# mikel-brostrom/boxmot

Hardware: NVIDIA H100
Metric: tracker.update() frames/sec at 256 dets/frame (higher is better)
Workload: dtype bf16x3

## Files before the change

boxmot_b200/csrc/reid_tc.cuh:

```cuda
#pragma once
#include "wgmma.cuh"

namespace bmb {
namespace tcx {

typedef __nv_bfloat16 bf16;

__device__ __forceinline__ int tc_chunk_count(const int* d_n, int off, int cap) {
    int n = *d_n - off;
    n = n < 0 ? 0 : n;
    return n > cap ? cap : n;
}
using um::mbar_arrive;

__global__ void k_maxpool_planes(const float* __restrict__ in, int H, int W, int C, const int* __restrict__ d_n, int off,
                                 int cap, bf16* __restrict__ out_hi, bf16* __restrict__ out_lo) {
    const int n_crops = tc_chunk_count(d_n, off, cap);
    const int OH = H / 2, OW = W / 2, C8 = C / 8;
    const size_t total = (size_t)n_crops * C8 * OH * OW;
    for (size_t e = (size_t)blockIdx.x * blockDim.x + threadIdx.x; e < total; e += (size_t)gridDim.x * blockDim.x) {
        const int ox = (int)(e % OW);
        size_t r = e / OW;
        const int oy = (int)(r % OH); r /= OH;
        const int c8 = (int)(r % C8);
// ... 448 lines not shown
};
inline GemmSmem gemm_smem_layout(int K8, int NP, int NP2, int n_stage, bool tail, bool pool, int slot_bytes, bool pool2 = false) {
    GemmSmem s{};
    size_t o = 0;
    s.b = o; o += (size_t)K8 * 2 * NP * 16;
    s.b2 = o; if (tail) o += (size_t)(NP / 8) * 2 * NP2 * 16;
    o = (o + 127) & ~(size_t)127;
    s.ring = o; o += (size_t)n_stage * slot_bytes;
    s.a2 = o;
    if (tail) {
        size_t a2 = (size_t)2 * (NP / 8) * 128 * 16;
        if (pool2) a2 = a2 > (size_t)128 * (NP2 + 4) * 4 ? a2 : (size_t)128 * (NP2 + 4) * 4;
        o += a2;
    }
    s.f = pool2 ? s.a2 : o;
    if (pool) o += (size_t)128 * (NP + 4) * 4;
    s.gate = o; o += 4 * 32 * 4 + 64;
    s.total = o + 128;
    return s;
}

enum GemmMode { GM_PLAIN, GM_POOL, GM_TAIL, GM_TAIL_POOL2, GM_HEAD };

template <int NP, int NP2, int MODE>
constexpr int gemm_min_ctas() {
    return NP == 128 || ((MODE == GM_TAIL || MODE == GM_TAIL_POOL2) && NP >= 96) ? 1 : 2;
}

template <int NP, int NP2, int MODE>
__global__ void __launch_bounds__(GEMM_THREADS, (gemm_min_ctas<NP, NP2, MODE>()))
    k_gemm_tc(const __grid_constant__ GemmTcArgs a, const int* __restrict__ d_n, int off, int cap, const GemmSmem L, const GemmHeadIO hio) {
    constexpr bool tail = MODE == GM_TAIL || MODE == GM_TAIL_POOL2, pool = MODE == GM_POOL, pool2 = MODE == GM_TAIL_POOL2;
    static_assert(NP % 16 == 0 && NP >= 16 && NP <= 128, "NP: 16 .. 128 output channels");
    static_assert(tail ? (NP2 % 16 == 0 && NP2 >= 16 && NP2 <= 128) : NP2 == 0, "NP2: the tail's output channels");
    constexpr int NACC = (NP2 > NP ? NP2 : NP) / 2;
    const int n = blockIdx.y;
    if (n >= tc_chunk_count(d_n, off, cap)) return;
    extern __shared__ __align__(128) unsigned char smem[];
    __shared__ __align__(8) uint64_t bar_full[4], bar_empty[4], bar_w;
    const int warp = threadIdx.x >> 5, lane = threadIdx.x & 31;
    const int tile0 = blockIdx.x * a.tiles_per_cta;
    const int tile1 = min(tile0 + a.tiles_per_cta, a.tiles_per_crop);
    unsigned char* sB = smem + L.b;
    unsigned char* sB2 = smem + L.b2;
    unsigned char* sRing = smem + L.ring;
    unsigned char* sA2 = smem + L.a2;
    float* sF = reinterpret_cast<float*>(smem + L.f);

    if (threadIdx.x == 0) {
        for (int i = 0; i < a.n_stage; ++i) { um::mbar_init(&bar_full[i], 1); um::mbar_init(&bar_empty[i], 2); }
        um::mbar_init(&bar_w, 1);
        um::fence_mbar_init();
    }
    __syncthreads();

    if (warp == 8) {
        if (lane == 0) {
            {
                const uint32_t first = (uint32_t)((a.bfold ? 4 * a.midp : 0) / 8) * 2u * NP * 16u, total = (uint32_t)a.K8 * 2u * NP * 16u;
                const uint32_t b2 = tail ? (uint32_t)(NP / 8) * 2u * NP2 * 16u : 0u;
                um::mbar_expect_tx(&bar_w, total + b2);
                if (first) um::bulk_g2s(sB, reinterpret_cast<const unsigned char*>(a.bfold) + (size_t)n * first, first, &bar_w);
                if (total > first) um::bulk_g2s(sB + first, reinterpret_cast<const unsigned char*>(a.b_packed) + first, total - first, &bar_w);
                if (b2) um::bulk_g2s(sB2, a.b2_packed, b2, &bar_w);
            }
            uint32_t it = 0;
            for (int tile = tile0; tile < tile1; ++tile) {
                for (int s = 0; s < a.n_src; ++s) {
                    const int kc = a.src_kc[s];
                    for (int p0 = 0; p0 < a.src_planes[s]; p0 += kc, ++it) {
                        const uint32_t slot = it % (uint32_t)a.n_stage, ph = (it / (uint32_t)a.n_stage) & 1u;
                        um::mbar_wait(&bar_empty[slot], ph ^ 1u);
                        unsigned char* dst = sRing + (size_t)slot * a.slot_bytes;
                        um::mbar_expect_tx(&bar_full[slot], (uint32_t)kc * 128u * 16u * 2u);
                        um::tma_load_4d(dst, &a.map_hi[s], 0, tile * 2, p0, n, &bar_full[slot]);
                        um::tma_load_4d(dst + a.slot_bytes / 2, &a.map_lo[s], 0, tile * 2, p0, n, &bar_full[slot]);
                    }
                }
            }
        }
        return;
    }

    const int et = threadIdx.x;
    const int wg = warp >> 2;
    const int row = wg * 64 + (warp & 3) * 16 + (lane >> 2);
    const int cq = 2 * (lane & 3);
    const uint32_t lbo_b = 2u * NP * 16u, lo_off = (uint32_t)NP * 16u;
    um::mbar_wait(&bar_w, 0);
    float acc[NACC];
    uint32_t it = 0;
    for (int tile = tile0; tile < tile1; ++tile) {
        uint32_t kplane = 0, first = 1;
        uint32_t held = 0;
        for (int s = 0; s < a.n_src; ++s) {
            const int kc = a.src_kc[s];
            for (int p0 = 0; p0 < a.src_planes[s]; p0 += kc, ++it) {
                const uint32_t slot = it % (uint32_t)a.n_stage, ph = (it / (uint32_t)a.n_stage) & 1u;
                um::mbar_wait(&bar_full[slot], ph);
                const uint32_t ah = um::smem_u32(sRing + (size_t)slot * a.slot_bytes) + (uint32_t)wg * 1024u, al = ah + a.slot_bytes / 2;
                for (int ks = 0; ks < kc / 2; ++ks) {
                    const uint32_t bb = um::smem_u32(sB) + (kplane + 2 * ks) * lbo_b;
                    const uint64_t xh = um::make_desc(ah + ks * 2 * 2048u, 2048u, 128), xl = um::make_desc(al + ks * 2 * 2048u, 2048u, 128);
                    um::wg_fence();
                    um::mma<NP, false>(acc, xh, bb, lbo_b, 128, first ? 0u : 1u);
                    um::mma<NP, false>(acc, xl, bb, lbo_b, 128, 1u);
                    um::mma<NP, false>(acc, xh, bb + lo_off, lbo_b, 128, 1u);
                    first = 0;
                    um::wg_commit();
                    um::wg_wait<1>();
                    if (ks == 0 && kplane > 0 && (et & 127) == 0) mbar_arrive(&bar_empty[held]);
                }
                held = slot;
                kplane += kc;
            }
        }
        um::wg_wait<0>();
        um::wg_fence_acc<NACC>(acc);
        if ((et & 127) == 0) mbar_arrive(&bar_empty[held]);
        if constexpr (MODE == GM_HEAD) {
            um::bar_sync(1, 256);
            float* part = reinterpret_cast<float*>(sRing);
            float* pooled = part + 8 * NP;
            float* red = pooled + NP;
            float* feat = red + 8;
#pragma unroll
            for (int i = 0; i < NP / 8; ++i) {
                const int c = 8 * i + cq;
                const float2 b = *reinterpret_cast<const float2*>(a.bias + c);
                float o0 = fmaxf(acc[4 * i] + b.x, 0.f) + fmaxf(acc[4 * i + 2] + b.x, 0.f);
                float o1 = fmaxf(acc[4 * i + 1] + b.y, 0.f) + fmaxf(acc[4 * i + 3] + b.y, 0.f);
#pragma unroll
                for (int sh = 4; sh < 32; sh <<= 1) {
                    o0 += __shfl_xor_sync(0xffffffffu, o0, sh);
                    o1 += __shfl_xor_sync(0xffffffffu, o1, sh);
                }
                if (lane < 4) *reinterpret_cast<float2*>(part + warp * NP + c) = make_float2(o0, o1);
            }
            um::bar_sync(1, 256);
            for (int c = et; c < NP; c += 256)
                pooled[c] = (((part[c] + part[NP + c]) + (part[2 * NP + c] + part[3 * NP + c])) +
                             ((part[4 * NP + c] + part[5 * NP + c]) + (part[6 * NP + c] + part[7 * NP + c]))) / 128.f;
            um::bar_sync(1, 256);
            const int FEAT = a.head_feat, C = a.N;
            float sq = 0.f;
            for (int f = et; f < FEAT; f += 256) {
                float t[8] = {0.f, 0.f, 0.f, 0.f, 0.f, 0.f, 0.f, 0.f};
                int c = 0;
                for (; c + 8 <= C; c += 8) {
#pragma unroll
                    for (int u = 0; u < 8; ++u) t[u] = fmaf(pooled[c + u], a.head_w[(size_t)(c + u) * FEAT + f], t[u]);
                }
                for (; c < C; ++c) t[0] = fmaf(pooled[c], a.head_w[(size_t)c * FEAT + f], t[0]);
                float sv = a.head_b[f] + (((t[0] + t[1]) + (t[2] + t[3])) + ((t[4] + t[5]) + (t[6] + t[7])));
                sv = fmaxf(sv, 0.f);
                feat[f] = sv;
                sq = fmaf(sv, sv, sq);
            }
#pragma unroll
            for (int sh = 16; sh > 0; sh >>= 1) sq += __shfl_xor_sync(0xffffffffu, sq, sh);
            if (lane == 0) red[warp] = sq;
            um::bar_sync(1, 256);
            float tot = 0.f;
            for (int w = 0; w < 8; ++w) tot += red[w];
            const float nrm = sqrtf(tot);
            float* dst = hio.out + (size_t)hio.crops[off + n].out_row * hio.out_ld;
            for (int f = et; f < FEAT; f += 256) dst[f] = feat[f] / nrm;
            um::bar_sync(1, 256);
        } else {
#pragma unroll
            for (int i = 0; i < NP / 8; ++i) {
                const int c = 8 * i + cq;
                const float2 b = *reinterpret_cast<const float2*>(a.bias + c);
#pragma unroll
                for (int h = 0; h < 2; ++h) {
                    const int m = row + 8 * h, px = tile * 128 + m;
                    float o0 = acc[4 * i + 2 * h] + b.x, o1 = acc[4 * i + 2 * h + 1] + b.y;
                    if (a.relu) { o0 = fmaxf(o0, 0.f); o1 = fmaxf(o1, 0.f); }
                    if (a.out_f32) {
                        float* dst = a.out_f32 + ((size_t)n * a.HW + px) * a.N + c;
                        if (c + 1 < a.N) *reinterpret_cast<float2*>(dst) = make_float2(o0, o1);
                        else if (c < a.N) dst[0] = o0;
                    }
                    if constexpr (pool) {
                        *reinterpret_cast<float2*>(sF + (size_t)m * (NP + 4) + c) = make_float2(o0, o1);
                    } else if (a.out_hi || tail) {
                        uint32_t hv, lv;
                        um::split2(o0, o1, hv, lv);
                        if (a.out_hi) {
                            const size_t e = (((size_t)n * (NP / 8) + i) * a.HW + px) * 4 + (lane & 3);
                            reinterpret_cast<uint32_t*>(a.out_hi)[e] = hv;
                            reinterpret_cast<uint32_t*>(a.out_lo)[e] = lv;
                        }
                        if constexpr (tail) {
                            *reinterpret_cast<uint32_t*>(sA2 + ((size_t)i * 128 + m) * 16 + (lane & 3) * 4) = hv;
                            *reinterpret_cast<uint32_t*>(sA2 + ((size_t)(NP / 8 + i) * 128 + m) * 16 + (lane & 3) * 4) = lv;
                        }
                    }
                }
            }
            auto pool_store = [&](const int NPx, bf16* o_hi, bf16* o_lo) {
                um::bar_sync(1, 256);
                const int Wt = a.W, OW = Wt / 2, OHt = a.rows_per_tile / 2;
                const int items = OHt * OW * (NPx / 8);
                const int OHW = a.HW / 4;
                for (int e = et; e < items; e += 256) {
                    const int pp = e % (OHt * OW), c8 = e / (OHt * OW);
                    const int oy = pp / OW, ox = pp - oy * OW;
                    const float* f0 = sF + (size_t)((2 * oy) * Wt + 2 * ox) * (NPx + 4) + c8 * 8;
                    const float* f1 = f0 + (NPx + 4);
                    const float* f2 = f0 + (size_t)Wt * (NPx + 4);
                    const float* f3 = f2 + (NPx + 4);
                    uint32_t h[4], l[4];
#pragma unroll
                    for (int j = 0; j < 4; ++j) {
                        const float x0 = (f0[2 * j] + f1[2 * j] + f2[2 * j] + f3[2 * j]) * 0.25f;
                        const float x1 = (f0[2 * j + 1] + f1[2 * j + 1] + f2[2 * j + 1] + f3[2 * j + 1]) * 0.25f;
                        um::split2(x0, x1, h[j], l[j]);
                    }
                    const int opx = (tile * OHt + oy) * OW + ox;
                    const size_t o = ((size_t)n * (NPx / 8) + c8) * OHW + opx;
                    reinterpret_cast<uint4*>(o_hi)[o] = make_uint4(h[0], h[1], h[2], h[3]);
                    reinterpret_cast<uint4*>(o_lo)[o] = make_uint4(l[0], l[1], l[2], l[3]);
                }
                um::bar_sync(1, 256);
            };
            if constexpr (pool) pool_store(NP, a.out_hi, a.out_lo);
            if constexpr (tail) {
                um::fence_async_smem();
                um::bar_sync(2 + wg, 128);
                const uint32_t lbo_b2 = 2u * NP2 * 16u, lo2 = (uint32_t)NP2 * 16u;
                const uint32_t ah = um::smem_u32(sA2) + (uint32_t)wg * 1024u, al = ah + (uint32_t)(NP / 8) * 2048u;
                um::wg_fence();
                for (int ks = 0; ks < NP / 16; ++ks) {
                    const uint32_t bb = um::smem_u32(sB2) + ks * 2 * lbo_b2;
                    const uint64_t xh = um::make_desc(ah + ks * 2 * 2048u, 2048u, 128), xl = um::make_desc(al + ks * 2 * 2048u, 2048u, 128);
                    um::mma<NP2, false>(acc, xh, bb, lbo_b2, 128, ks > 0);
                    um::mma<NP2, false>(acc, xl, bb, lbo_b2, 128, 1u);
                    um::mma<NP2, false>(acc, xh, bb + lo2, lbo_b2, 128, 1u);
                }
                um::wg_commit();
                um::wg_wait<0>();
                um::wg_fence_acc<NACC>(acc);
                if constexpr (pool2) um::bar_sync(1, 256);
#pragma unroll
                for (int i = 0; i < NP2 / 8; ++i) {
                    const int c = 8 * i + cq;
                    const float2 b = *reinterpret_cast<const float2*>(a.bias2 + c);
#pragma unroll
                    for (int h = 0; h < 2; ++h) {
                        const int m = row + 8 * h, px = tile * 128 + m;
                        const float o0 = fmaxf(acc[4 * i + 2 * h] + b.x, 0.f), o1 = fmaxf(acc[4 * i + 2 * h + 1] + b.y, 0.f);
                        if constexpr (pool2) {
                            *reinterpret_cast<float2*>(sF + (size_t)m * (NP2 + 4) + c) = make_float2(o0, o1);
                        } else {
                            uint32_t hv, lv;
                            um::split2(o0, o1, hv, lv);
                            const size_t e = (((size_t)n * (NP2 / 8) + i) * a.HW + px) * 4 + (lane & 3);
                            reinterpret_cast<uint32_t*>(a.out2_hi)[e] = hv;
                            reinterpret_cast<uint32_t*>(a.out2_lo)[e] = lv;
                        }
                    }
                }
                if constexpr (pool2) pool_store(NP2, a.out2_hi, a.out2_lo);
            }
        }
    }
}

typedef void (*GemmKernel)(GemmTcArgs, const int*, int, int, GemmSmem, GemmHeadIO);
struct GemmInstance { int NP, NP2, mode; GemmKernel fn; };
#define BMB_GEMM(np, np2, mode) {np, np2, mode, k_gemm_tc<np, np2, mode>}
static const GemmInstance kGemmInstances[] = {
    BMB_GEMM(16, 0, GM_PLAIN), BMB_GEMM(32, 0, GM_PLAIN),
    BMB_GEMM(64, 0, GM_PLAIN), BMB_GEMM(96, 0, GM_PLAIN),
    BMB_GEMM(128, 0, GM_PLAIN),
    BMB_GEMM(64, 0, GM_POOL), BMB_GEMM(96, 0, GM_POOL),
    BMB_GEMM(64, 16, GM_TAIL), BMB_GEMM(96, 32, GM_TAIL), BMB_GEMM(128, 32, GM_TAIL),
    BMB_GEMM(64, 64, GM_TAIL_POOL2), BMB_GEMM(96, 96, GM_TAIL_POOL2),
    BMB_GEMM(128, 0, GM_HEAD),
};
#undef BMB_GEMM
inline GemmKernel gemm_instance(int NP, int NP2, int mode) {
    for (const GemmInstance& g : kGemmInstances)
        if (g.NP == NP && g.NP2 == NP2 && g.mode == mode) return g.fn;
    return nullptr;
}


struct FrontTcArgs {
    const uint8_t* images;
    size_t image_stride;
    int rows, cols;
    const void* crops;
    const bf16* w;
    const float* bias_tab;
    bf16* p_hi;
    bf16* p_lo;
    float* dbg_crop;
    int pad_mode;
};
struct FrontCrop { float x1, y1, x2, y2; int image, out_row; };

constexpr int FR_COLS = 39, FR_ROWS = 264, FR_CS = FR_ROWS * 8 + 16;
constexpr int FR_A_BYTES = FR_COLS * FR_CS;
constexpr int FR_W_BYTES = 7 * 4 * 32 * 16;
constexpr int FR_H_BYTES = 4 * 128 * 16 * 4;
constexpr size_t FR_SMEM = FR_A_BYTES + FR_W_BYTES + FR_H_BYTES + 128;

__device__ __forceinline__ void fr_coeff(int d, int src_n, double scale, bool clamp, int& idx, int& a0, int& a1) {
    float f = (float)(((double)d + 0.5) * scale - 0.5);
    int s = (int)floorf(f);
    f = f - (float)s;
    if (clamp) {
        if (s < 0) { s = 0; f = 0.f; }
        if (s >= src_n - 1) { s = src_n - 1; f = 0.f; }
    }
    idx = s;
    a0 = (int)rintf((1.0f - f) * 2048.0f);
    a1 = (int)rintf(f * 2048.0f);
}

__global__ void __launch_bounds__(256, 1) k_front_tc(const FrontTcArgs a, const int* __restrict__ d_n, int off, int cap) {
    const int n = blockIdx.y;
    if (n >= tc_chunk_count(d_n, off, cap)) return;
    const int strip = blockIdx.x;
    extern __shared__ __align__(128) unsigned char smem[];
    __shared__ int xi[128], xa0[128], xa1[128], yi[256], ya0[256], ya1[256];
    __shared__ __align__(16) float sBias[4 * 4 * 16];
    unsigned char* sA = smem;
    unsigned char* sW = smem + FR_A_BYTES;
    float* sH = reinterpret_cast<float*>(smem + FR_A_BYTES + FR_W_BYTES);
    const int warp = threadIdx.x >> 5, lane = threadIdx.x & 31;
    const FrontCrop cd = reinterpret_cast<const FrontCrop*>(a.crops)[off + n];
#ifdef BMB_TC_CLOCKS
    long long fk[16];
    int nfk = 0;
#define FCK() do { if (threadIdx.x == 0 && nfk < 16) fk[nfk++] = clock64(); } while (0)
#else
#define FCK() do { } while (0)
#endif
    FCK();

    const int x1 = (int)rintf(cd.x1), y1 = (int)rintf(cd.y1), x2 = (int)rintf(cd.x2), y2 = (int)rintf(cd.y2);
    const int cx1 = max(0, x1), cy1 = max(0, y1), cx2 = min(a.cols, x2), cy2 = min(a.rows, y2);
    const bool valid = cx2 > cx1 && cy2 > cy1;
    const int sw = cx2 - cx1, sh = cy2 - cy1;
    int nw = 128, nh = 256, pl = 0, pt = 0;
    if (valid && a.pad_mode) {
        const double sc = fmin(128.0 / (double)sw, 256.0 / (double)sh);
        nw = max(1, (int)((double)sw * sc));
        nh = max(1, (int)((double)sh * sc));
        pl = (128 - nw) / 2;
        pt = (256 - nh) / 2;
    }
    if (valid) {
        const double sx = 1.0 / ((double)nw / (double)sw), sy = 1.0 / ((double)nh / (double)sh);
        for (int d = threadIdx.x; d < nw; d += 256) fr_coeff(d, sw, sx, true, xi[d], xa0[d], xa1[d]);
        for (int d = threadIdx.x; d < nh; d += 256) fr_coeff(d, sh, sy, false, yi[d], ya0[d], ya1[d]);
    }
    for (int e = threadIdx.x; e < FR_A_BYTES / 16; e += 256) reinterpret_cast<uint4*>(sA)[e] = make_uint4(0u, 0u, 0u, 0u);
    for (int e = threadIdx.x; e < FR_W_BYTES / 16; e += 256) reinterpret_cast<uint4*>(sW)[e] = reinterpret_cast<const uint4*>(a.w)[e];
    for (int e = threadIdx.x; e < 256; e += 256) sBias[e] = a.bias_tab[e];
    __syncthreads();
    FCK();
    const int xin0 = 32 * strip - 5;
    if (valid) {
        const uint8_t* img = a.images + (size_t)cd.image * a.image_stride;
        for (int base = threadIdx.x; base < 40 * 256; base += 4 * 256) {
            int h0[4][3], h1[4][3], bb0[4], bb1[4], so[4];
            bool ok[4], border[4];
#pragma unroll
            for (int u = 0; u < 4; ++u) {
                const int p = base + u * 256;
                const int dy = p / 40, lc = p - dy * 40;
                const int dx = xin0 + lc;
                ok[u] = p < 40 * 256 && lc < FR_COLS && dx >= 0 && dx < 128;
                const int ry = dy - pt, rx = dx - pl;
                border[u] = rx < 0 || rx >= nw || ry < 0 || ry >= nh;
                const int dxc = min(max(rx, 0), nw - 1), dyc = min(max(ry, 0), nh - 1);
                const int sx0 = xi[dxc], sx1 = min(sx0 + 1, sw - 1);
                const int r0 = min(max(yi[dyc], 0), sh - 1), r1 = min(max(yi[dyc] + 1, 0), sh - 1);
                const uint8_t* p0 = img + ((size_t)(cy1 + r0) * a.cols + cx1) * 3;
                const uint8_t* p1 = img + ((size_t)(cy1 + r1) * a.cols + cx1) * 3;
                const int a0 = xa0[dxc], a1 = xa1[dxc];
                bb0[u] = ya0[dyc]; bb1[u] = ya1[dyc];
                so[u] = lc * FR_CS + (min(dy, 255) + 3) * 8;
#pragma unroll
                for (int c = 0; c < 3; ++c) {
                    h0[u][c] = (int)__ldg(p0 + sx0 * 3 + c) * a0 + (int)__ldg(p0 + sx1 * 3 + c) * a1;
                    h1[u][c] = (int)__ldg(p1 + sx0 * 3 + c) * a0 + (int)__ldg(p1 + sx1 * 3 + c) * a1;
                }
            }
#pragma unroll
            for (int u = 0; u < 4; ++u) {
                if (!ok[u]) continue;
                int v[3];
#pragma unroll
                for (int c = 0; c < 3; ++c) {
                    const int r = (((bb0[u] * (h0[u][c] >> 4)) >> 16) + ((bb1[u] * (h1[u][c] >> 4)) >> 16) + 2) >> 2;
                    v[c] = min(max(r, 0), 255);
                }
                if (border[u]) { v[0] = 104; v[1] = 116; v[2] = 124; }
                const __nv_bfloat162 rg = __floats2bfloat162_rn((float)v[2], (float)v[1]);
                const __nv_bfloat162 b_ = __floats2bfloat162_rn((float)v[0], 0.f);
                *reinterpret_cast<uint2*>(sA + so[u]) = make_uint2(*reinterpret_cast<const uint32_t*>(&rg), *reinterpret_cast<const uint32_t*>(&b_));
                if (a.dbg_crop) {
                    const int p = base + u * 256;
                    const int dy = p / 40, dx = xin0 + (p - dy * 40);
                    float* o = a.dbg_crop + (((size_t)n * 256 + dy) * 128 + dx) * 3;
                    o[0] = (float)v[2]; o[1] = (float)v[1]; o[2] = (float)v[0];
                }
            }
        }
    } else if (a.dbg_crop) {
        for (int p = threadIdx.x; p < 40 * 256; p += 256) {
            const int dy = p / 40, lc = p - dy * 40;
            const int dx = xin0 + lc;
            if (lc < FR_COLS && dx >= 0 && dx < 128) {
                float* o = a.dbg_crop + (((size_t)n * 256 + dy) * 128 + dx) * 3;
                o[0] = 0.f; o[1] = 0.f; o[2] = 0.f;
            }
        }
    }
    um::fence_async_smem();
    __syncthreads();
    FCK();

    const int wg = warp >> 2;
    const int row = wg * 64 + (warp & 3) * 16 + (lane >> 2);
    const int cq = 2 * (lane & 3);
    int rcl[2];
#pragma unroll
    for (int h = 0; h < 2; ++h) {
        const int oy = row + 8 * h;
        rcl[h] = oy == 0 ? 0 : (oy == 1 ? 1 : (oy == 127 ? 3 : 2));
    }
    float prev1[2][4], prev2[2][4];
#pragma unroll
    for (int h = 0; h < 2; ++h)
#pragma unroll
        for (int c = 0; c < 4; ++c) { prev1[h][c] = 0.f; prev2[h][c] = 0.f; }
    const uint32_t sa = um::smem_u32(sA) + (uint32_t)wg * 1024u, sw_ = um::smem_u32(sW);
    for (int j0 = 0; j0 < 17; j0 += 8) {
        const int j1 = min(j0 + 8, 17);
        for (int j = j0; j < j1; ++j) {
            const int ox = 16 * strip - 1 + j;
            float v[2][4];
            if (ox >= 0) {
                float acc[16];
                um::wg_fence();
#pragma unroll
                for (int kx = 0; kx < 7; ++kx)
#pragma unroll
                    for (int ks = 0; ks < 2; ++ks)
                        um::mma<32, false>(acc, um::make_desc(sa + (uint32_t)(2 * j + kx) * FR_CS + ks * 32, 16, 128),
                                           sw_ + (uint32_t)(kx * 4 + 2 * ks) * 512u, 512u, 128, (kx | ks) != 0);
                um::wg_commit();
                um::wg_wait_all();
                um::wg_fence_acc<16>(acc);
                const int cc = ox == 0 ? 0 : (ox == 1 ? 1 : (ox == 63 ? 3 : 2));
#pragma unroll
                for (int h = 0; h < 2; ++h) {
                    const float* bb = sBias + (rcl[h] * 4 + cc) * 16;
#pragma unroll
                    for (int i = 0; i < 2; ++i)
#pragma unroll
                        for (int e = 0; e < 2; ++e)
                            v[h][2 * i + e] = fmaxf(acc[4 * i + 2 * h + e] + acc[4 * (i + 2) + 2 * h + e] + bb[8 * i + cq + e], 0.f);
                }
            } else {
#pragma unroll
                for (int h = 0; h < 2; ++h)
#pragma unroll
                    for (int c = 0; c < 4; ++c) v[h][c] = 0.f;
            }
            if ((j & 1) == 0 && j >= 2) {
                float* hs = sH + (size_t)(((j - j0) >> 1) & 3) * 128 * 16;
#pragma unroll
                for (int h = 0; h < 2; ++h)
#pragma unroll
                    for (int i = 0; i < 2; ++i)
                        *reinterpret_cast<float2*>(hs + (row + 8 * h) * 16 + 8 * i + cq) =
                            make_float2(fmaxf(fmaxf(prev2[h][2 * i], prev1[h][2 * i]), v[h][2 * i]),
                                        fmaxf(fmaxf(prev2[h][2 * i + 1], prev1[h][2 * i + 1]), v[h][2 * i + 1]));
            }
#pragma unroll
            for (int h = 0; h < 2; ++h)
#pragma unroll
                for (int c = 0; c < 4; ++c) { prev2[h][c] = prev1[h][c]; prev1[h][c] = v[h][c]; }
        }
        __syncthreads();
        const int s_first = j0 == 0 ? 1 : 0, s_last = j0 == 0 ? 3 : (j0 == 8 ? 3 : 0);
        const int items = (s_last - s_first + 1) * 64 * 2;
        for (int e = threadIdx.x; e < items; e += 256) {
            const int s = s_first + (e >> 7), py = (e >> 1) & 63, half = e & 1;
            const float* hs = sH + (size_t)s * 128 * 16 + half * 8;
            const int oy = 2 * py;
            float m[8];
#pragma unroll
            for (int c = 0; c < 8; ++c) {
                const float up = oy > 0 ? hs[(oy - 1) * 16 + c] : 0.f;
                m[c] = fmaxf(fmaxf(up, hs[oy * 16 + c]), hs[(oy + 1) * 16 + c]);
            }
            const int px = 8 * strip + (j0 + 2 * s) / 2 - 1;
            uint32_t h4[4], l4[4];
#pragma unroll
            for (int c = 0; c < 4; ++c) um::split2(m[2 * c], m[2 * c + 1], h4[c], l4[c]);
            const size_t o = (((size_t)n * 2 + half) * 64 + py) * 32 + px;
            reinterpret_cast<uint4*>(a.p_hi)[o] = make_uint4(h4[0], h4[1], h4[2], h4[3]);
            reinterpret_cast<uint4*>(a.p_lo)[o] = make_uint4(l4[0], l4[1], l4[2], l4[3]);
        }
        __syncthreads();
        FCK();
    }
#ifdef BMB_TC_CLOCKS
    if (threadIdx.x == 0 && n == 5) {
        printf("front strip %d: setup %lld resize %lld |", strip, fk[1] - fk[0], fk[2] - fk[1]);
        for (int i = 3; i < nfk; ++i) printf(" batch %lld |", fk[i] - fk[i - 1]);
        printf(" total %lld\n", fk[nfk - 1] - fk[0]);
    }
#endif
}

}
}
```

boxmot_b200/csrc/reid_tc_plan.cuh:

```cuda
#pragma once

namespace bmb {
namespace tcx {

struct ChainShape { int CP, CR, W, H, R, kind; };
static const ChainShape kChainShapes[3] = {{16, 16, 32, 64, chain_rows<BMB_CHAIN_S2>(), LK_CHAIN_S2}, {32, 24, 16, 32, chain_rows<BMB_CHAIN_S3>(), LK_CHAIN_S3},
                                           {32, 32, 8, 16, chain_rows<BMB_CHAIN_S4>(), LK_CHAIN_S4}};

inline bool plan_supported(const ReidModel* m) {
    return m->arch == 1 && m->c[0] == 16 && m->c[1] == 64 && m->c[2] == 96 && m->c[3] == 128;
}

Plan* plan_build(ReidModel* m, const float* hw) {
    Plan* P = new Plan();
    try {
        P->chunk = m->chunk;
        const size_t CH = (size_t)m->chunk;
        int dev = 0;
        RCUDA_OK(cudaGetDevice(&dev));
        RCUDA_OK(cudaDeviceGetAttribute(&P->smem_limit, cudaDevAttrMaxSharedMemoryPerBlockOptin, dev));
        P->smem_limit -= 1024;
        alloc_planes(P->P, CH * 2048 * 16);
        alloc_planes(P->X1, CH * 2048 * 16);
        alloc_planes(P->Y, CH * 2048 * 64);
        alloc_planes(P->XA, CH * 2048 * 64);
        alloc_planes(P->XB, CH * 2048 * 64);
        RCUDA_OK(cudaMalloc(&P->c5, sizeof(float) * CH * 128 * m->c[3]));
        for (int b = 0; b < 4; ++b) RCUDA_OK(cudaMalloc(&P->sums[b], sizeof(float) * CH * 8 * 32));
        RCUDA_OK(cudaMalloc(&P->gates, sizeof(float) * CH * 4 * 32));
        RCUDA_OK(cudaMalloc(&P->arrivals, sizeof(int) * CH));
        RCUDA_OK(cudaMemset(P->arrivals, 0, sizeof(int) * CH));
        RCUDA_OK(cudaMalloc(&P->bfold, (size_t)CH * 16 * 2 * 128 * 16));
        RCUDA_OK(cudaMalloc(&P->dbg, sizeof(float) * CH * 2048 * 64));

        std::vector<uint16_t> wb;
        std::vector<float> wf;
        struct BlkOff { size_t pw[10], dw[10], lb[10], c1, c1b, cx, cxb; } bo[6];
        for (int bi = 0; bi < 6; ++bi) {
            const BlockW& b = m->blocks[bi];
            const int midp = pad16(b.mid);
            for (int l = 0; l < 10; ++l) {
                bo[bi].pw[l] = pack_b(wb, hw + b.light[l].pw, b.mid, b.mid, b.mid, midp / 8, midp);
                size_t at = (wf.size() + 3) / 4 * 4;
                wf.resize(at + 9 * midp, 0.f);
                for (int t = 0; t < 9; ++t)
                    for (int c = 0; c < b.mid; ++c) wf[at + t * midp + c] = hw[b.light[l].dw + (size_t)t * b.mid + c];
                bo[bi].dw[l] = at;
                bo[bi].lb[l] = pack_f(wf, hw + b.light[l].b, b.mid, midp);
                if (bo[bi].lb[l] != at + (size_t)9 * midp) throw std::runtime_error("chain weights: taps and bias are not contiguous");
            }
            bo[bi].c1 = pack_b(wb, hw + b.c1w, b.cin, b.mid, b.mid, b.cin / 8, midp);
            bo[bi].c1b = pack_f(wf, hw + b.c1b, b.mid, midp);
            const int K8 = 4 * midp / 8 + b.cin / 8;
            if (b.has_ds)
                bo[bi].cx = pack_b(wb, hw + b.cw + (size_t)b.mid * b.cout, b.cin, b.cout, b.cout, K8, b.cout, 4 * midp);
            else
                bo[bi].cx = pack_b(wb, nullptr, b.cin, b.cout, b.cout, K8, b.cout, 4 * midp, true);
            bo[bi].cxb = pack_f(wf, hw + b.cb, b.cout, b.cout);
        }
        size_t tr[2], trb[2];
        for (int s = 0; s < 2; ++s) {
            const int C = m->c[s + 1];
            tr[s] = pack_b(wb, hw + m->trans_w[s], C, C, C, C / 8, C);
            trb[s] = pack_f(wf, hw + m->trans_b[s], C, C);
        }
        const size_t c5 = pack_b(wb, hw + m->c5w, m->c[3], m->c[3], m->c[3], m->c[3] / 8, m->c[3]);
        const size_t c5b = pack_f(wf, hw + m->c5b, m->c[3], m->c[3]);
        size_t fw, fb;
        {
            const double mean[3] = {0.485, 0.456, 0.406}, stdv[3] = {0.229, 0.224, 0.225};
            const int C0 = m->c[0];
            fw = (wb.size() + 63) / 64 * 64;
            wb.resize(fw + 7 * 4 * 32 * 8, 0);
            for (int kx = 0; kx < 7; ++kx)
                for (int ky = 0; ky < 7; ++ky)
                    for (int ci = 0; ci < 3; ++ci)
                        for (int co = 0; co < C0; ++co) {
                            const float v = (float)((double)hw[m->stem_w + (size_t)((ky * 7 + kx) * 3 + ci) * C0 + co] / (255.0 * stdv[ci]));
                            const int k = ky * 4 + ci;
                            uint16_t* plane = wb.data() + fw + ((size_t)(kx * 4 + k / 8) * 32) * 8;
                            const uint16_t h = f2bf(v);
                            plane[(size_t)co * 8 + k % 8] = h;
                            plane[(size_t)(16 + co) * 8 + k % 8] = f2bf(v - bf2f(h));
                        }
            fb = (wf.size() + 3) / 4 * 4;
            wf.resize(fb + 4 * 4 * 16, 0.f);
            const int lo_[4] = {3, 1, 0, 0}, hi_[4] = {6, 6, 6, 4};
            for (int rc = 0; rc < 4; ++rc)
                for (int cc = 0; cc < 4; ++cc)
                    for (int co = 0; co < C0; ++co) {
                        double acc = hw[m->stem_b + co];
                        for (int ky = lo_[rc]; ky <= hi_[rc]; ++ky)
                            for (int kx = lo_[cc]; kx <= hi_[cc]; ++kx)
                                for (int ci = 0; ci < 3; ++ci)
                                    acc -= (double)hw[m->stem_w + (size_t)((ky * 7 + kx) * 3 + ci) * C0 + co] * mean[ci] / stdv[ci];
                        wf[fb + (rc * 4 + cc) * 16 + co] = (float)acc;
                    }
        }
        RCUDA_OK(cudaMalloc(&P->d_wb, wb.size() * 2 + 256));
        RCUDA_OK(cudaMemcpy(P->d_wb, wb.data(), wb.size() * 2, cudaMemcpyHostToDevice));
        RCUDA_OK(cudaMalloc(&P->d_wf, wf.size() * 4 + 256));
        RCUDA_OK(cudaMemcpy(P->d_wf, wf.data(), wf.size() * 4, cudaMemcpyHostToDevice));
        const bf16* WB = P->d_wb;
        const float* WF = P->d_wf;
        const float* W32 = m->d_w;

        RCUDA_OK(chain_prepare<BMB_CHAIN_S2>());
        RCUDA_OK(chain_prepare<BMB_CHAIN_S3>());
        RCUDA_OK(chain_prepare<BMB_CHAIN_S4>());
        for (const GemmInstance& gi : kGemmInstances)
            RCUDA_OK(cudaFuncSetAttribute(gi.fn, cudaFuncAttributeMaxDynamicSharedMemorySize, P->smem_limit));
        RCUDA_OK(cudaFuncSetAttribute(k_front_tc, cudaFuncAttributeMaxDynamicSharedMemorySize, (int)FR_SMEM));

        struct Src { Planes* buf; int C8; };
        auto gemm = [&](int H, int Wd, std::vector<Src> srcs, size_t b_off, int N, size_t bias_off, bool relu) -> Launch {
            Launch L{};
            L.kind = LK_GEMM;
            L.cls = CLS_POINTWISE;
            GemmTcArgs& g = L.gemm;
            g.n_src = (int)srcs.size();
            g.rows_per_tile = 128 / Wd;
            g.tiles_per_crop = H * Wd / 128;
            g.tiles_per_cta = g.tiles_per_crop >= 16 ? 4 : (g.tiles_per_crop >= 4 ? 2 : 1);
            g.K8 = 0;
            for (int s = 0; s < g.n_src; ++s) {
                const int C8 = srcs[s].C8;
                const int kc = C8 % 4 == 0 ? 4 : 2;
                g.src_planes[s] = C8;
                g.src_kc[s] = kc;
                g.K8 += C8;
                L.src_hi[s] = srcs[s].buf->hi;
                L.src_lo[s] = srcs[s].buf->lo;
            }
            g.b_packed = WB + b_off;
            g.N = N;
            g.NP = pad16(N);
            g.bias = WF + bias_off;
            g.relu = relu ? 1 : 0;
            g.HW = H * Wd;
            g.W = Wd;
            return L;
        };
        auto finish_into = [&](Launch& L, std::vector<Launch>* out) {
            GemmTcArgs& g = L.gemm;
            const bool tail = g.b2_packed != nullptr;
            if (g.NP > 128 || (tail && g.NP2 > 128)) throw std::runtime_error("tensor-core GEMM: more than 128 output channels");
            const int mode = g.head_w ? GM_HEAD : g.pool ? GM_POOL : !tail ? GM_PLAIN : g.pool2 ? GM_TAIL_POOL2 : GM_TAIL;
            L.gemm_fn = gemm_instance(g.NP, tail ? g.NP2 : 0, mode);
            if (!L.gemm_fn)
                throw std::runtime_error("tensor-core GEMM: no kernel instance for NP = " + std::to_string(g.NP) + ", NP2 = " +
                                         std::to_string(tail ? g.NP2 : 0) + ", epilogue mode " + std::to_string(mode));
            auto layout = [&](int ns) { return gemm_smem_layout(g.K8, g.NP, g.NP2, ns, tail, g.pool != 0, g.slot_bytes, g.pool2 != 0); };
            auto ctas = [&](int ns) {
                const size_t bytes = layout(ns).total;
                int c = 0;
                if ((int)bytes <= P->smem_limit)
                    RCUDA_OK(cudaOccupancyMaxActiveBlocksPerMultiprocessor(&c, L.gemm_fn, GEMM_THREADS, bytes));
                return c;
            };
            int ns = 0;
            for (int pass = 0; pass < 2 && !ns; ++pass) {
                int kc_max = 2;
                for (int s = 0; s < g.n_src; ++s) {
                    if (pass == 1) g.src_kc[s] = 2;
                    kc_max = std::max(kc_max, g.src_kc[s]);
                }
                g.slot_bytes = kc_max * 128 * 16 * 2;
                for (int cand = 4; cand >= 2 && !ns; --cand)
                    if (ctas(cand) >= 2) ns = cand;
            }
            if (!ns) {
                int kc_max = 2;
                for (int s = 0; s < g.n_src; ++s) {
                    g.src_kc[s] = g.src_planes[s] % 4 == 0 ? 4 : 2;
                    kc_max = std::max(kc_max, g.src_kc[s]);
                }
                g.slot_bytes = kc_max * 128 * 16 * 2;
                for (int cand = 4; cand >= 2 && !ns; --cand)
                    if (ctas(cand) >= 1) ns = cand;
            }
            if (!ns) throw std::runtime_error("tensor-core GEMM does not fit shared memory");
            L.gemm_ctas = ctas(ns);
            for (int s = 0; s < g.n_src; ++s) {
                make_tile_map(&g.map_hi[s], L.src_hi[s], P->chunk, g.src_planes[s], g.HW, g.src_kc[s]);
                make_tile_map(&g.map_lo[s], L.src_lo[s], P->chunk, g.src_planes[s], g.HW, g.src_kc[s]);
            }
            L.gl = layout(ns);
            g.n_stage = ns;
            L.gemm_groups = (g.tiles_per_crop + g.tiles_per_cta - 1) / g.tiles_per_cta;
            out->push_back(L);
        };
        auto dbg = [&](Launch& L, int stage, const Planes& buf, int C8, int HW, int C) {
            L.stage_after = stage;
            L.dbg_hi = buf.hi; L.dbg_lo = buf.lo; L.dbg_C8 = C8; L.dbg_HW = HW; L.dbg_C = C;
        };

        auto build_launches = [&](bool fuse_trans, std::vector<Launch>* out) {
            auto finish = [&](Launch& L) { finish_into(L, out); };
        {
            Launch L{};
            L.kind = LK_FRONT;
            L.cls = CLS_STEM;
            L.front.w = WB + fw;
            L.front.bias_tab = WF + fb;
            L.front.p_hi = P->P.hi; L.front.p_lo = P->P.lo;
            dbg(L, 2, P->P, 2, 2048, 16);
            out->push_back(L);
        }
        Planes* X = &P->P;
        Planes* Xo = &P->XA;
        Planes* Xspare = &P->XB;
        int xC8 = 2;
        int H = 64, Wd = 32;
        int stage = 3;
        {
            const BlockW& b = m->blocks[0];
            Launch L = gemm(H, Wd, {{X, xC8}}, bo[0].c1, b.mid, bo[0].c1b, true);
            L.gemm.out_hi = P->X1.hi; L.gemm.out_lo = P->X1.lo;
            dbg(L, 100, P->X1, pad16(b.mid) / 8, H * Wd, pad16(b.mid));
            finish(L);
        }
        for (int s = 0; s < 3; ++s) {
            const ChainShape& cs = kChainShapes[s];
            bool trans_done = false;
            for (int j = 0; j < 2; ++j) {
                const int bi = s * 2 + j;
                const BlockW& b = m->blocks[bi];
                const int midp = pad16(b.mid);
                {
                    Launch L{};
                    L.kind = cs.kind;
                    L.cls = CLS_LIGHTCONV;
                    ChainTcArgs& c = L.chain;
                    make_rows_map(&c.map_hi, P->X1.hi, P->chunk, midp / 8, H, Wd, cs.R + 8);
                    make_rows_map(&c.map_lo, P->X1.lo, P->chunk, midp / 8, H, Wd, cs.R + 8);
                    for (int l = 0; l < 10; ++l) {
                        c.wpw[l] = WB + bo[bi].pw[l];
                        c.wdw[l] = WF + bo[bi].dw[l];
                        c.bias[l] = WF + bo[bi].lb[l];
                    }
                    c.y_hi = P->Y.hi; c.y_lo = P->Y.lo;
                    for (int br = 0; br < 4; ++br) c.sums[br] = P->sums[br];
                    c.H = H;
                    GatesTcArgs& ga = c.gate;
                    for (int br = 0; br < 4; ++br) ga.sums[br] = P->sums[br];
                    ga.g1w = W32 + b.g1w; ga.g1b = W32 + b.g1b; ga.g2w = W32 + b.g2w; ga.g2b = W32 + b.g2b;
                    ga.gates = P->gates;
                    ga.mid = b.mid; ga.midp = midp; ga.hid = b.hid; ga.tiles = H / cs.R; ga.HW = H * Wd;
                    ga.w3 = W32 + b.cw; ga.bfold = P->bfold; ga.N = b.cout; ga.NP = pad16(b.cout);
                    ga.arrivals = P->arrivals;
                    L.chain_tiles = H / cs.R;
                    dbg(L, 200 + bi, P->Y, 4 * midp / 8, H * Wd, 4 * midp);
                    out->push_back(L);
                }
                {
                    Launch L = gemm(H, Wd, {{&P->Y, 4 * midp / 8}, {X, xC8}}, bo[bi].cx, b.cout, bo[bi].cxb, true);
                    GemmTcArgs& g = L.gemm;
                    g.bfold = P->bfold;
                    g.midp = midp;
                    g.out_hi = Xo->hi; g.out_lo = Xo->lo;
                    bool fused_trans = false;
                    if (j == 0) {
                        const BlockW& nb = m->blocks[bi + 1];
                        const int nmidp = pad16(nb.mid);
                        const GemmSmem probe = gemm_smem_layout(g.K8, g.NP, nmidp, 2, true, false, 4 * 128 * 16 * 2);
                        if ((int)probe.total <= P->smem_limit) {
                            g.b2_packed = WB + bo[bi + 1].c1;
                            g.bias2 = WF + bo[bi + 1].c1b;
                            g.N2 = nb.mid; g.NP2 = nmidp;
                            g.out2_hi = P->X1.hi; g.out2_lo = P->X1.lo;
                        }
                    } else if (s < 2 && fuse_trans) {
                        const int C = m->c[s + 1];
                        const GemmSmem probe = gemm_smem_layout(g.K8, g.NP, C, 2, true, false, 2 * 128 * 16 * 2, true);
                        if ((int)probe.total <= P->smem_limit && g.NP + C <= 512) {
                            g.b2_packed = WB + tr[s];
                            g.bias2 = WF + trb[s];
                            g.N2 = C; g.NP2 = C;
                            g.pool2 = 1;
                            g.out_hi = nullptr; g.out_lo = nullptr;
                            g.out2_hi = Xo->hi; g.out2_lo = Xo->lo;
                            fused_trans = true;
                        }
                    }
                    if (fused_trans) {
                        ++stage;
                        dbg(L, stage++, *Xo, m->c[s + 1] / 8, H * Wd / 4, m->c[s + 1]);
                    } else {
                        dbg(L, stage++, *Xo, b.cout / 8, H * Wd, b.cout);
                    }
                    const bool fused_next = g.b2_packed != nullptr && !fused_trans;
                    finish(L);
                    Planes* t = X == &P->P ? Xspare : X;
                    X = Xo; Xo = t; xC8 = b.cout / 8;
                    trans_done = fused_trans;
                    if (j == 0 && !fused_next) {
                        const BlockW& nb = m->blocks[bi + 1];
                        Launch L2 = gemm(H, Wd, {{X, xC8}}, bo[bi + 1].c1, nb.mid, bo[bi + 1].c1b, true);
                        L2.gemm.out_hi = P->X1.hi; L2.gemm.out_lo = P->X1.lo;
                        dbg(L2, 100 + bi + 1, P->X1, pad16(nb.mid) / 8, H * Wd, pad16(nb.mid));
                        finish(L2);
                    }
                }
            }
            if (s < 2) {
                const int C = m->c[s + 1];
                if (!trans_done) {
                    Launch L = gemm(H, Wd, {{X, xC8}}, tr[s], C, trb[s], true);
                    L.gemm.pool = 1;
                    L.gemm.out_hi = Xo->hi; L.gemm.out_lo = Xo->lo;
                    dbg(L, stage++, *Xo, C / 8, H * Wd / 4, C);
                    finish(L);
                    Planes* t = X; X = Xo; Xo = t;
                }
                H /= 2; Wd /= 2;
                const BlockW& nb = m->blocks[(s + 1) * 2];
                Launch L = gemm(H, Wd, {{X, xC8}}, bo[(s + 1) * 2].c1, nb.mid, bo[(s + 1) * 2].c1b, true);
                L.gemm.out_hi = P->X1.hi; L.gemm.out_lo = P->X1.lo;
                dbg(L, 100 + (s + 1) * 2, P->X1, pad16(nb.mid) / 8, H * Wd, pad16(nb.mid));
                finish(L);
            }
        }
        {
            Launch L = gemm(H, Wd, {{X, xC8}}, c5, m->c[3], c5b, true);
            if (fuse_trans && H * Wd == 128) {
                L.gemm.head_w = W32 + m->fcw;
                L.gemm.head_b = W32 + m->fcb;
                L.gemm.head_feat = m->feat;
                L.cls = CLS_HEAD;
                P->head_fused = true;
            } else {
                L.gemm.out_f32 = P->c5;
            }
            L.stage_after = 11;
            finish(L);
        }
        };
        build_launches(true, &P->launches);
        build_launches(false, &P->launches_dbg);
    } catch (...) {
        plan_free(P);
        throw;
    }
    return P;
}

struct FrontInput { const uint8_t* images; size_t image_stride; int rows, cols; const CropDesc* crops; float* out; int out_ld; };

template <class Prof>
int plan_run(ReidModel* m, const FrontInput& fi, const int* d_n, int off, int upper, cudaStream_t st, bool* stopped, Prof& prof) {
    Plan* P = m->tc;
    int launches = 0;
    for (const Launch& L : (m->debug_stop >= 0 ? P->launches_dbg : P->launches)) {
        prof.begin(L.cls);
        switch (L.kind) {
            case LK_FRONT: {
                FrontTcArgs fa = L.front;
                fa.images = fi.images; fa.image_stride = fi.image_stride; fa.rows = fi.rows; fa.cols = fi.cols; fa.crops = fi.crops;
                fa.pad_mode = m->preprocess;
                if (m->debug_stop == 50) {
                    if (!P->dbg_crop) RCUDA_OK(cudaMalloc(&P->dbg_crop, sizeof(float) * (size_t)P->chunk * 256 * 128 * 3));
                    fa.dbg_crop = P->dbg_crop;
                }
                k_front_tc<<<dim3(4, upper), 256, FR_SMEM, st>>>(fa, d_n, off, upper);
                break;
            }
            case LK_MAXPOOL_PLANES:
                k_maxpool_planes<<<m->sms * 4, 256, 0, st>>>(m->bufA, 128, 64, m->c[0], d_n, off, upper, P->P.hi, P->P.lo);
                break;
            case LK_CHAIN_S2:
                chain_launch<BMB_CHAIN_S2>(L.chain, L.chain_tiles, upper, d_n, off, st);
                break;
            case LK_CHAIN_S3:
                chain_launch<BMB_CHAIN_S3>(L.chain, L.chain_tiles, upper, d_n, off, st);
                break;
            case LK_CHAIN_S4:
                chain_launch<BMB_CHAIN_S4>(L.chain, L.chain_tiles, upper, d_n, off, st);
                break;
            case LK_GEMM:
                L.gemm_fn<<<dim3(L.gemm_groups, upper), GEMM_THREADS, L.gl.total, st>>>(L.gemm, d_n, off, upper, L.gl, GemmHeadIO{fi.crops, fi.out, fi.out_ld});
                break;
        }
        prof.end();
        ++launches;
        if (m->debug_stop == 50 && L.kind == LK_FRONT) {
            m->debug_ptr = P->dbg_crop;
            m->debug_floats_per_crop = (size_t)256 * 128 * 3;
            *stopped = true;
            return launches;
        }
        if (m->debug_stop >= 0 && L.stage_after == m->debug_stop) {
            if (L.stage_after == 11) {
                m->debug_ptr = P->c5;
                m->debug_floats_per_crop = (size_t)128 * m->c[3];
            } else {
                k_planes_to_nhwc<<<m->sms * 4, 256, 0, st>>>(L.dbg_hi, L.dbg_lo, L.dbg_C8, L.dbg_HW, L.dbg_C, d_n, off, upper, P->dbg);
                m->debug_ptr = P->dbg;
                m->debug_floats_per_crop = (size_t)L.dbg_HW * L.dbg_C;
            }
            *stopped = true;
            return launches;
        }
    }
    return launches;
}

}
}
```

Measured before the change: 708.1.

## Narrow front-stem strips to raise occupancy and double-buffer stem WGMMA

Splits the fused resize/stem/pool front kernel into 8 narrower column strips instead of 4, shrinking per-CTA shared memory so two CTAs fit per SM (launch bounds and an occupancy check enforce this). The stem convolution now double-buffers WGMMA accumulators so the next column's MMA overlaps the current column's bias/ReLU epilogue, and pooling runs once at the end with vectorized float4 reads. The zero-fill of the staging buffer only covers columns and halo rows that the resize does not overwrite. The trade is more halo recomputation across strips and higher register pressure from two accumulator sets.

Result: no change. 713.4, median of 6 (+0.8%).

```diff
diff --git a/boxmot_b200/csrc/reid_tc.cuh b/boxmot_b200/csrc/reid_tc.cuh
--- a/boxmot_b200/csrc/reid_tc.cuh
+++ b/boxmot_b200/csrc/reid_tc.cuh
@@ -774,11 +774,16 @@
 };
 struct FrontCrop { float x1, y1, x2, y2; int image, out_row; };
 
-constexpr int FR_COLS = 39, FR_ROWS = 264, FR_CS = FR_ROWS * 8 + 16;
+constexpr int FR_STRIPS = 8, FR_PX = 4, FR_J = 2 * FR_PX + 1;
+constexpr int FR_COLS = 4 * FR_PX + 7, FR_ROWS = 264, FR_CS = FR_ROWS * 8 + 16;
+constexpr int FR_LANES = FR_COLS + 1;
+constexpr int FR_U = 6;
 constexpr int FR_A_BYTES = FR_COLS * FR_CS;
 constexpr int FR_W_BYTES = 7 * 4 * 32 * 16;
-constexpr int FR_H_BYTES = 4 * 128 * 16 * 4;
+constexpr int FR_H_BYTES = FR_PX * 128 * 16 * 4;
 constexpr size_t FR_SMEM = FR_A_BYTES + FR_W_BYTES + FR_H_BYTES + 128;
+static_assert(FR_STRIPS * FR_PX == 32, "the strips cover the 32 pooled columns");
+static_assert(FR_LANES * 256 % (FR_U * 256) == 0, "whole resize rounds");
 
 __device__ __forceinline__ void fr_coeff(int d, int src_n, double scale, bool clamp, int& idx, int& a0, int& a1) {
     float f = (float)(((double)d + 0.5) * scale - 0.5);
@@ -793,7 +798,18 @@
     a1 = (int)rintf(f * 2048.0f);
 }
 
-__global__ void __launch_bounds__(256, 1) k_front_tc(const FrontTcArgs a, const int* __restrict__ d_n, int off, int cap) {
+__device__ __forceinline__ void fr_stem_mma(float* d, uint32_t sa, uint32_t sw, int j) {
+    um::wg_fence();
+#pragma unroll
+    for (int kx = 0; kx < 7; ++kx)
+#pragma unroll
+        for (int ks = 0; ks < 2; ++ks)
+            um::mma<32, false>(d, um::make_desc(sa + (uint32_t)(2 * j + kx) * FR_CS + ks * 32, 16, 128),
+                               sw + (uint32_t)(kx * 4 + 2 * ks) * 512u, 512u, 128, (kx | ks) != 0);
+    um::wg_commit();
+}
+
+__global__ void __launch_bounds__(256, 2) k_front_tc(const FrontTcArgs a, const int* __restrict__ d_n, int off, int cap) {
     const int n = blockIdx.y;
     if (n >= tc_chunk_count(d_n, off, cap)) return;
     const int strip = blockIdx.x;
@@ -806,9 +822,9 @@
     const int warp = threadIdx.x >> 5, lane = threadIdx.x & 31;
     const FrontCrop cd = reinterpret_cast<const FrontCrop*>(a.crops)[off + n];
 #ifdef BMB_TC_CLOCKS
-    long long fk[16];
+    long long fk[8];
     int nfk = 0;
-#define FCK() do { if (threadIdx.x == 0 && nfk < 16) fk[nfk++] = clock64(); } while (0)
+#define FCK() do { if (threadIdx.x == 0 && nfk < 8) fk[nfk++] = clock64(); } while (0)
 #else
 #define FCK() do { } while (0)
 #endif
@@ -831,23 +847,30 @@
         for (int d = threadIdx.x; d < nw; d += 256) fr_coeff(d, sw, sx, true, xi[d], xa0[d], xa1[d]);
         for (int d = threadIdx.x; d < nh; d += 256) fr_coeff(d, sh, sy, false, yi[d], ya0[d], ya1[d]);
     }
-    for (int e = threadIdx.x; e < FR_A_BYTES / 16; e += 256) reinterpret_cast<uint4*>(sA)[e] = make_uint4(0u, 0u, 0u, 0u);
+    const int xin0 = 4 * FR_PX * strip - 5;
+    const int zc0 = valid ? min(max(-xin0, 0), FR_COLS) : FR_COLS;
+    const int zc1 = valid ? max(min(128 - xin0, FR_COLS), zc0) : FR_COLS;
+    for (int e = threadIdx.x; e < zc0 * (FR_CS / 16); e += 256) reinterpret_cast<uint4*>(sA)[e] = make_uint4(0u, 0u, 0u, 0u);
+    for (int e = zc1 * (FR_CS / 16) + threadIdx.x; e < FR_A_BYTES / 16; e += 256) reinterpret_cast<uint4*>(sA)[e] = make_uint4(0u, 0u, 0u, 0u);
+    for (int e = threadIdx.x; e < (zc1 - zc0) * 10; e += 256) {
+        const int c = zc0 + e / 10, r = e - (e / 10) * 10;
+        *reinterpret_cast<uint2*>(sA + c * FR_CS + (r < 3 ? r : 256 + r) * 8) = make_uint2(0u, 0u);
+    }
     for (int e = threadIdx.x; e < FR_W_BYTES / 16; e += 256) reinterpret_cast<uint4*>(sW)[e] = reinterpret_cast<const uint4*>(a.w)[e];
     for (int e = threadIdx.x; e < 256; e += 256) sBias[e] = a.bias_tab[e];
     __syncthreads();
     FCK();
-    const int xin0 = 32 * strip - 5;
     if (valid) {
         const uint8_t* img = a.images + (size_t)cd.image * a.image_stride;
-        for (int base = threadIdx.x; base < 40 * 256; base += 4 * 256) {
-            int h0[4][3], h1[4][3], bb0[4], bb1[4], so[4];
-            bool ok[4], border[4];
-#pragma unroll
-            for (int u = 0; u < 4; ++u) {
+        for (int base = threadIdx.x; base < FR_LANES * 256; base += FR_U * 256) {
+            int h0[FR_U][3], h1[FR_U][3], bb0[FR_U], bb1[FR_U], so[FR_U];
+            bool ok[FR_U], border[FR_U];
+#pragma unroll
+            for (int u = 0; u < FR_U; ++u) {
                 const int p = base + u * 256;
-                const int dy = p / 40, lc = p - dy * 40;
+                const int dy = p / FR_LANES, lc = p - dy * FR_LANES;
                 const int dx = xin0 + lc;
-                ok[u] = p < 40 * 256 && lc < FR_COLS && dx >= 0 && dx < 128;
+                ok[u] = lc < FR_COLS && dx >= 0 && dx < 128;
                 const int ry = dy - pt, rx = dx - pl;
                 border[u] = rx < 0 || rx >= nw || ry < 0 || ry >= nh;
                 const int dxc = min(max(rx, 0), nw - 1), dyc = min(max(ry, 0), nh - 1);
@@ -857,7 +880,7 @@
                 const uint8_t* p1 = img + ((size_t)(cy1 + r1) * a.cols + cx1) * 3;
                 const int a0 = xa0[dxc], a1 = xa1[dxc];
                 bb0[u] = ya0[dyc]; bb1[u] = ya1[dyc];
-                so[u] = lc * FR_CS + (min(dy, 255) + 3) * 8;
+                so[u] = lc * FR_CS + (dy + 3) * 8;
 #pragma unroll
                 for (int c = 0; c < 3; ++c) {
                     h0[u][c] = (int)__ldg(p0 + sx0 * 3 + c) * a0 + (int)__ldg(p0 + sx1 * 3 + c) * a1;
@@ -865,7 +888,7 @@
                 }
             }
 #pragma unroll
-            for (int u = 0; u < 4; ++u) {
+            for (int u = 0; u < FR_U; ++u) {
                 if (!ok[u]) continue;
                 int v[3];
 #pragma unroll
@@ -879,15 +902,15 @@
                 *reinterpret_cast<uint2*>(sA + so[u]) = make_uint2(*reinterpret_cast<const uint32_t*>(&rg), *reinterpret_cast<const uint32_t*>(&b_));
                 if (a.dbg_crop) {
                     const int p = base + u * 256;
-                    const int dy = p / 40, dx = xin0 + (p - dy * 40);
+                    const int dy = p / FR_LANES, dx = xin0 + (p - dy * FR_LANES);
                     float* o = a.dbg_crop + (((size_t)n * 256 + dy) * 128 + dx) * 3;
                     o[0] = (float)v[2]; o[1] = (float)v[1]; o[2] = (float)v[0];
                 }
             }
         }
     } else if (a.dbg_crop) {
-        for (int p = threadIdx.x; p < 40 * 256; p += 256) {
-            const int dy = p / 40, lc = p - dy * 40;
+        for (int p = threadIdx.x; p < FR_LANES * 256; p += 256) {
+            const int dy = p / FR_LANES, lc = p - dy * FR_LANES;
             const int dx = xin0 + lc;
             if (lc < FR_COLS && dx >= 0 && dx < 128) {
                 float* o = a.dbg_crop + (((size_t)n * 256 + dy) * 128 + dx) * 3;
@@ -914,84 +937,67 @@
 #pragma unroll
         for (int c = 0; c < 4; ++c) { prev1[h][c] = 0.f; prev2[h][c] = 0.f; }
     const uint32_t sa = um::smem_u32(sA) + (uint32_t)wg * 1024u, sw_ = um::smem_u32(sW);
-    for (int j0 = 0; j0 < 17; j0 += 8) {
-        const int j1 = min(j0 + 8, 17);
-        for (int j = j0; j < j1; ++j) {
-            const int ox = 16 * strip - 1 + j;
-            float v[2][4];
-            if (ox >= 0) {
-                float acc[16];
-                um::wg_fence();
-#pragma unroll
-                for (int kx = 0; kx < 7; ++kx)
-#pragma unroll
-                    for (int ks = 0; ks < 2; ++ks)
-                        um::mma<32, false>(acc, um::make_desc(sa + (uint32_t)(2 * j + kx) * FR_CS + ks * 32, 16, 128),
-                                           sw_ + (uint32_t)(kx * 4 + 2 * ks) * 512u, 512u, 128, (kx | ks) != 0);
-                um::wg_commit();
-                um::wg_wait_all();
-                um::wg_fence_acc<16>(acc);
-                const int cc = ox == 0 ? 0 : (ox == 1 ? 1 : (ox == 63 ? 3 : 2));
-#pragma unroll
-                for (int h = 0; h < 2; ++h) {
-                    const float* bb = sBias + (rcl[h] * 4 + cc) * 16;
-#pragma unroll
-                    for (int i = 0; i < 2; ++i)
-#pragma unroll
-                        for (int e = 0; e < 2; ++e)
-                            v[h][2 * i + e] = fmaxf(acc[4 * i + 2 * h + e] + acc[4 * (i + 2) + 2 * h + e] + bb[8 * i + cq + e], 0.f);
-                }
-            } else {
-#pragma unroll
-                for (int h = 0; h < 2; ++h)
-#pragma unroll
-                    for (int c = 0; c < 4; ++c) v[h][c] = 0.f;
-            }
-            if ((j & 1) == 0 && j >= 2) {
-                float* hs = sH + (size_t)(((j - j0) >> 1) & 3) * 128 * 16;
-#pragma unroll
-                for (int h = 0; h < 2; ++h)
-#pragma unroll
-                    for (int i = 0; i < 2; ++i)
-                        *reinterpret_cast<float2*>(hs + (row + 8 * h) * 16 + 8 * i + cq) =
-                            make_float2(fmaxf(fmaxf(prev2[h][2 * i], prev1[h][2 * i]), v[h][2 * i]),
-                                        fmaxf(fmaxf(prev2[h][2 * i + 1], prev1[h][2 * i + 1]), v[h][2 * i + 1]));
-            }
+    float acc[2][16];
+    fr_stem_mma(acc[0], sa, sw_, 0);
+#pragma unroll
+    for (int j = 0; j < FR_J; ++j) {
+        float* cur = acc[j & 1];
+        if (j + 1 < FR_J) {
+            fr_stem_mma(acc[(j + 1) & 1], sa, sw_, j + 1);
+            um::wg_wait<1>();
+        } else {
+            um::wg_wait<0>();
+        }
+        um::wg_fence_acc<16>(cur);
+        const int ox = 2 * FR_PX * strip - 1 + j;
+        const int cc = ox <= 0 ? 0 : (ox == 1 ? 1 : (ox == 63 ? 3 : 2));
+        float v[2][4];
+#pragma unroll
+        for (int h = 0; h < 2; ++h) {
+            const float* bb = sBias + (rcl[h] * 4 + cc) * 16;
+#pragma unroll
+            for (int i = 0; i < 2; ++i)
+#pragma unroll
+                for (int e = 0; e < 2; ++e) {
+                    const float x = fmaxf(cur[4 * i + 2 * h + e] + cur[4 * (i + 2) + 2 * h + e] + bb[8 * i + cq + e], 0.f);
+                    v[h][2 * i + e] = ox >= 0 ? x : 0.f;
+                }
+        }
+        if ((j & 1) == 0 && j >= 2) {
+            float* hs = sH + (size_t)(j / 2 - 1) * 128 * 16;
 #pragma unroll
             for (int h = 0; h < 2; ++h)
 #pragma unroll
-                for (int c = 0; c < 4; ++c) { prev2[h][c] = prev1[h][c]; prev1[h][c] = v[h][c]; }
-        }
-        __syncthreads();
-        const int s_first = j0 == 0 ? 1 : 0, s_last = j0 == 0 ? 3 : (j0 == 8 ? 3 : 0);
-        const int items = (s_last - s_first + 1) * 64 * 2;
-        for (int e = threadIdx.x; e < items; e += 256) {
-            const int s = s_first + (e >> 7), py = (e >> 1) & 63, half = e & 1;
-            const float* hs = sH + (size_t)s * 128 * 16 + half * 8;
-            const int oy = 2 * py;
-            float m[8];
-#pragma unroll
-            for (int c = 0; c < 8; ++c) {
-                const float up = oy > 0 ? hs[(oy - 1) * 16 + c] : 0.f;
-                m[c] = fmaxf(fmaxf(up, hs[oy * 16 + c]), hs[(oy + 1) * 16 + c]);
-            }
-            const int px = 8 * strip + (j0 + 2 * s) / 2 - 1;
-            uint32_t h4[4], l4[4];
-#pragma unroll
-            for (int c = 0; c < 4; ++c) um::split2(m[2 * c], m[2 * c + 1], h4[c], l4[c]);
-            const size_t o = (((size_t)n * 2 + half) * 64 + py) * 32 + px;
-            reinterpret_cast<uint4*>(a.p_hi)[o] = make_uint4(h4[0], h4[1], h4[2], h4[3]);
-            reinterpret_cast<uint4*>(a.p_lo)[o] = make_uint4(l4[0], l4[1], l4[2], l4[3]);
-        }
-        __syncthreads();
-        FCK();
-    }
+                for (int i = 0; i < 2; ++i)
+                    *reinterpret_cast<float2*>(hs + (row + 8 * h) * 16 + 8 * i + cq) =
+                        make_float2(fmaxf(fmaxf(prev2[h][2 * i], prev1[h][2 * i]), v[h][2 * i]),
+                                    fmaxf(fmaxf(prev2[h][2 * i + 1], prev1[h][2 * i + 1]), v[h][2 * i + 1]));
+        }
+#pragma unroll
+        for (int h = 0; h < 2; ++h)
+#pragma unroll
+            for (int c = 0; c < 4; ++c) { prev2[h][c] = prev1[h][c]; prev1[h][c] = v[h][c]; }
+    }
+    FCK();
+    __syncthreads();
+    for (int e = threadIdx.x; e < FR_PX * 64 * 4; e += 256) {
+        const int s = e >> 8, py = (e >> 2) & 63, c4 = e & 3;
+        const float4* hs = reinterpret_cast<const float4*>(sH + (size_t)s * 128 * 16) + c4;
+        const int oy = 2 * py;
+        const float4 u = oy > 0 ? hs[(oy - 1) * 4] : make_float4(0.f, 0.f, 0.f, 0.f), c = hs[oy * 4], d = hs[(oy + 1) * 4];
+        uint32_t h2[2], l2[2];
+        um::split2(fmaxf(fmaxf(u.x, c.x), d.x), fmaxf(fmaxf(u.y, c.y), d.y), h2[0], l2[0]);
+        um::split2(fmaxf(fmaxf(u.z, c.z), d.z), fmaxf(fmaxf(u.w, c.w), d.w), h2[1], l2[1]);
+        const int px = FR_PX * strip + s;
+        const size_t o = ((((size_t)n * 2 + (c4 >> 1)) * 64 + py) * 32 + px) * 2 + (c4 & 1);
+        reinterpret_cast<uint2*>(a.p_hi)[o] = make_uint2(h2[0], h2[1]);
+        reinterpret_cast<uint2*>(a.p_lo)[o] = make_uint2(l2[0], l2[1]);
+    }
+    FCK();
 #ifdef BMB_TC_CLOCKS
-    if (threadIdx.x == 0 && n == 5) {
-        printf("front strip %d: setup %lld resize %lld |", strip, fk[1] - fk[0], fk[2] - fk[1]);
-        for (int i = 3; i < nfk; ++i) printf(" batch %lld |", fk[i] - fk[i - 1]);
-        printf(" total %lld\n", fk[nfk - 1] - fk[0]);
-    }
+    if (threadIdx.x == 0 && n == 5)
+        printf("front strip %d: setup %lld resize %lld stem %lld pool %lld | total %lld\n", strip, fk[1] - fk[0], fk[2] - fk[1],
+               fk[3] - fk[2], fk[4] - fk[3], fk[4] - fk[0]);
 #endif
 }
 
diff --git a/boxmot_b200/csrc/reid_tc_plan.cuh b/boxmot_b200/csrc/reid_tc_plan.cuh
--- a/boxmot_b200/csrc/reid_tc_plan.cuh
+++ b/boxmot_b200/csrc/reid_tc_plan.cuh
@@ -111,6 +111,11 @@
         for (const GemmInstance& gi : kGemmInstances)
             RCUDA_OK(cudaFuncSetAttribute(gi.fn, cudaFuncAttributeMaxDynamicSharedMemorySize, P->smem_limit));
         RCUDA_OK(cudaFuncSetAttribute(k_front_tc, cudaFuncAttributeMaxDynamicSharedMemorySize, (int)FR_SMEM));
+        {
+            int c = 0;
+            RCUDA_OK(cudaOccupancyMaxActiveBlocksPerMultiprocessor(&c, k_front_tc, 256, FR_SMEM));
+            if (c < 2) throw std::runtime_error("k_front_tc: " + std::to_string(c) + " CTA(s) per SM, laid out for 2");
+        }
 
         struct Src { Planes* buf; int C8; };
         auto gemm = [&](int H, int Wd, std::vector<Src> srcs, size_t b_off, int N, size_t bias_off, bool relu) -> Launch {
@@ -362,7 +367,7 @@
                     if (!P->dbg_crop) RCUDA_OK(cudaMalloc(&P->dbg_crop, sizeof(float) * (size_t)P->chunk * 256 * 128 * 3));
                     fa.dbg_crop = P->dbg_crop;
                 }
-                k_front_tc<<<dim3(4, upper), 256, FR_SMEM, st>>>(fa, d_n, off, upper);
+                k_front_tc<<<dim3(FR_STRIPS, upper), 256, FR_SMEM, st>>>(fa, d_n, off, upper);
                 break;
             }
             case LK_MAXPOOL_PLANES:
```
